# esw0116/DynaVSR

Hardware: AMD Instinct MI355X
Metric: inner-loop frames/sec/GPU (EDVR-M x4, 5x3x180x320): forward leg = BASELINE.json configs[1]; the inner MAML step and the per-frame pipeline are `inner_step` / `per_frame_pipeline` (higher is better)
Workload: dtype f32; 1 GPU; EDVR-M x4 forward (PCD deformable alignment + TSA fusion + reconstruction), clips of 1x5x3x180x320 -> 3x720x1280 (BASELINE.json configs[1]); one step = 2 clip(s) per GPU, one per HIP stream (adapt.super_resolve_video); clips_in_flight_per_gpu=2

## Files before the change

dynavsr_amd/_lib.py:

```python
import ctypes
import os
from ctypes import POINTER, Structure, c_char_p, c_float, c_int, c_longlong, c_size_t, c_void_p

import torch

_runtime = {"configured": False, "hw_queues": None, "effective": None}


def configure_runtime(hw_queues=6):
    if not _runtime["configured"]:
        user = os.environ.get("GPU_MAX_HW_QUEUES")
        late = torch.cuda.is_initialized()
        if user is None and not late:
            os.environ["GPU_MAX_HW_QUEUES"] = str(int(hw_queues))
        _runtime.update(configured=True, hw_queues=os.environ.get("GPU_MAX_HW_QUEUES"),
                        effective=(user is not None) or not late)
    return {"hw_queues": _runtime["hw_queues"], "effective": _runtime["effective"]}


def runtime_report(device=None):
    r = configure_runtime()
    overlaps = None
    if torch.cuda.is_available():
        with torch.cuda.device(device if device is not None else torch.cuda.current_device()):
# ... 101 lines not shown
        "dvsr_conv2d_backward": (I, [POINTER(Conv2dDesc), P, P, P, P, P, P, c_size_t, P]),
        "dvsr_mdcn_backward_workspace_bytes": (c_size_t, [I] * 10),
        "dvsr_mdcn_backward": (I, [P] * 10 + [I] * 12 + [P, c_size_t, P]),
        "dvsr_adam_step": (I, [POINTER(c_void_p)] * 4 + [POINTER(LL), I, F, F, F, F, F, I, P]),
        "dvsr_sgd_step": (I, [POINTER(c_void_p)] * 2 + [POINTER(LL), I, F, F, P]),
        "dvsr_replicate_tensors": (I, [POINTER(c_void_p)] * 2 + [POINTER(LL), I, I, P]),
        "dvsr_degrade_apply": (I, [P, P, P, I, I, I, I, I, I, I, I, I, P]),
        "dvsr_frame_metrics_workspace_bytes": (c_size_t, [I, I, I]),
        "dvsr_frame_metrics": (I, [P, P, I, I, I, F, F, P, P, P, c_size_t, P]),
        "dvsr_charbonnier_workspace_bytes": (c_size_t, []),
        "dvsr_charbonnier_forward": (I, [P, P, P, LL, F, P, c_size_t, P]),
        "dvsr_conv2d_packed_workspace_bytes": (c_size_t, [POINTER(Conv2dDesc)]),
        "dvsr_conv2d_forward_packed": (I, [POINTER(Conv2dDesc), P, c_size_t, P]),
        "dvsr_conv2d_dgrad_packed": (I, [POINTER(Conv2dDesc), P, P, P, c_size_t, P]),
        "dvsr_conv2d_packed_geometry": (I, [POINTER(Conv2dDesc), POINTER(ctypes.c_int * 4)]),
        "dvsr_conv2d_wgrad_geometry": (I, [POINTER(Conv2dDesc), I, I, POINTER(ctypes.c_int * 8)]),
        "dvsr_conv2d_wgrad_workspace_bytes": (c_size_t, [POINTER(Conv2dDesc), I]),
        "dvsr_conv2d_wgrad_bf16": (I, [POINTER(Conv2dDesc), P, P, P, P, c_size_t, P]),
        "dvsr_conv2d_wgrad_split3": (I, [POINTER(Conv2dDesc), P, P, P, P, c_size_t, P]),
        "dvsr_flow_warp_forward": (I, [P, P, P, I, I, I, I, LL, P]),
        "dvsr_flow_warp_backward": (I, [P, P, P, P, P, I, I, I, I, LL, P]),
        "dvsr_avgpool2_forward": (I, [P, P, LL, I, I, P]),
        "dvsr_avgpool2_backward": (I, [P, P, LL, I, I, I, P]),
        "dvsr_resize_bilinear_ac_forward": (I, [P, P, LL, I, I, I, I, F, LL, P]),
        "dvsr_resize_bilinear_ac_backward": (I, [P, P, LL, I, I, I, I, F, LL, P]),
        "dvsr_upsample_bicubic_ac_forward": (I, [P, P, LL, I, I, I, P]),
        "dvsr_upsample_bicubic_ac_backward": (I, [P, P, LL, I, I, I, P]),
        "dvsr_channel_affine": (I, [P, P, P, P, I, I, LL, LL, LL, I, P]),
        "dvsr_batchnorm_workspace_bytes": (c_size_t, [I]),
        "dvsr_batchnorm_forward": (I, [P] * 8 + [I, I, LL, I, F, F, I, P, c_size_t, P]),
# ... 10 lines not shown
        "dvsr_l1_tail_backward": (I, [P, P, P, F, P, LL, P]),
        "dvsr_charbonnier_backward": (I, [P, P, P, P, LL, F, P]),
        "dvsr_charbonnier_forward_grouped": (I, [P, P, P, LL, I, F, P, c_size_t, P]),
        "dvsr_charbonnier_backward_grouped": (I, [P, P, P, P, LL, I, F, P]),
        "dvsr_l1_tail_forward_grouped": (I, [P, P, P, F, P, LL, I, P, c_size_t, P]),
        "dvsr_l1_tail_backward_grouped": (I, [P, P, P, F, P, LL, I, P]),
        "dvsr_edvr_op_info": (I, [P, I, c_char_p, I, c_char_p, I, POINTER(ctypes.c_double),
                                  POINTER(ctypes.c_double)]),
        "dvsr_edvr_forward_timed": (I, [P, POINTER(c_void_p), P, P, P, c_size_t, P, POINTER(c_float)]),
        "dvsr_debug_mfma_peak": (LL, [P, I, I, I, I, P]),
        "dvsr_debug_mfma_shadow": (I, [P, P, I, I, I, I, I, P]),
        "dvsr_edvr_tensor_info": (I, [P, c_char_p, POINTER(LL), POINTER(LL)]),
        "dvsr_edvr_plan_work": (I, [P, POINTER(ctypes.c_double * 9)]),
        "dvsr_edvr_plan_work_nograd": (I, [P, POINTER(ctypes.c_double * 9)]),
        "dvsr_edvr_op_launch_count": (I, [P, I, I]),
        "dvsr_side_stream_overlaps": (I, [P]),
        "dvsr_edvr_op_output": (I, [P, I, I, POINTER(c_int), POINTER(LL), POINTER(LL)]),
        "dvsr_estimator_plan_work": (I, [P, POINTER(ctypes.c_double * 9)]),
        "dvsr_edvr_stream_create": (I, [POINTER(EdvrConfig), I, I, I, POINTER(c_void_p)]),
        "dvsr_edvr_stream_destroy": (None, [P]),
        "dvsr_edvr_stream_num_params": (I, [P]),
        "dvsr_edvr_stream_num_launches": (I, [P, I]),
        "dvsr_edvr_stream_cache_bytes": (c_size_t, [P]),
        "dvsr_edvr_stream_workspace_bytes": (c_size_t, [P]),
        "dvsr_edvr_stream_extract": (I, [P, POINTER(c_void_p), P, I, P, c_size_t, P, c_size_t, I, P]),
        "dvsr_edvr_stream_fuse": (I, [P, POINTER(c_void_p), POINTER(c_int), P, c_size_t, P, P, c_size_t, I, P]),
        "dvsr_frame_ingest": (I, [P, POINTER(FrameDesc), P, I, I, I, P]),
        "dvsr_frame_emit": (I, [P, I, I, P, POINTER(FrameDesc), F, F, P]),
        "dvsr_edvr_stream_extract_frame": (I, [P, POINTER(c_void_p), P, POINTER(FrameDesc), I, I, P, c_size_t, P, c_size_t, I,
                                               P]),
# ... 52 lines not shown
```

dynavsr_amd/csrc/conv2d_v2.hip:

```cpp
#include <algorithm>
#include <cmath>
#include <cstdlib>
#include <type_traits>

#include "common.h"
#include "kernels.h"
#include "small_grid.h"

namespace dvsr {

#ifdef DVSR_CONV_TRACE
#define DVSR_ABLATE(a) ((a).ablate)
#define DVSR_STAMP(i)                                                                              \
  do {                                                                                             \
    if (a.trace && threadIdx.x == 0) a.trace[(size_t)blockIdx.x * 64 + (i)] = __builtin_readcyclecounter(); \
  } while (0)
#else
#define DVSR_ABLATE(a) 0
#define DVSR_STAMP(i) \
  do {                \
  } while (0)
#endif

template <int KS, int S, int CC, int TH, int MT, int BF = 0>
struct Conv2Shape {
  static constexpr int TW = 32, KK = KS * KS, NT = TH / 4;
  static constexpr int IH = (TH - 1) * S + KS, IW = (TW - 1) * S + KS;
  static constexpr int PLANE = IH * IW, E = (PLANE + 255) / 256;
  static constexpr int KQ4 = BF ? CC / 16 : CC / 8;
  static constexpr int PIECES = BF == 2 ? 3 : 1;
  static constexpr int IN1 = KQ4 * PLANE * 8;
  static constexpr int IN_FLOATS = PIECES * IN1;
  static constexpr int HALF = KK * KQ4 * 2 * 32 * 4;
  static constexpr int W1 = MT * HALF;
  static constexpr bool AG = BF == 2;
  static constexpr int W_FLOATS = AG ? 0 : PIECES * W1;
  static constexpr int NPIECE = W_FLOATS / 256;
  static constexpr int BUF_FLOATS = IN_FLOATS + W_FLOATS;
  static constexpr size_t LDS_BYTES = (size_t)2 * BUF_FLOATS * sizeof(float);
};

__global__ void pack_weights_kernel(PackTable t) {
  const PackEntry& e = t.e[blockIdx.y];
  if (e.bf || has_own_pack_kernel(e.layout)) return;
  const int kq4 = e.CC / 8;
  const size_t per_chunk = (size_t)e.pch;
  const size_t total = (size_t)e.ncb * e.nchunks * per_chunk;
  for (size_t i = blockIdx.x * (size_t)blockDim.x + threadIdx.x; i < total;
       i += (size_t)gridDim.x * blockDim.x) {
    int r = (int)(i % per_chunk);
    const size_t ck = i / per_chunk;
    const int k = (int)(ck % e.nchunks), cb = (int)(ck / e.nchunks);
    const int j = r & 3; r >>= 2;
    const int lo = r & 31; r >>= 5;
// ... 100 lines not shown
  const int wave = __builtin_amdgcn_readfirstlane(tid >> 6);
  const int lo = lane & 31, hi = lane >> 5;
  const int Ctot = a.c0 + a.c1;
  const size_t HW = (size_t)a.H * a.W;
  const float* x0n = a.x0 + (size_t)n * a.x0_bs;
  const float* x1n = a.c1 ? a.x1 + (size_t)(n / a.x1_bdiv) * a.x1_bs : x0n;
  const size_t cstride0 = a.in_dil ? (size_t)a.Hs * a.Ws : HW;

  unsigned eoffb[E];
  int elds[E];
  bool evalid[E];
#pragma unroll
  for (int e = 0; e < E; ++e) {
    const int idx = tid + 256 * e;
    const int iy = idx / IW, ix = idx - iy * IW;
    elds[e] = (iy * 2) * IW + ix;
    const int gy = iy0 + iy, gx = ix0 + ix;
    bool ok = idx < PLANE && (unsigned)gy < (unsigned)a.H && (unsigned)gx < (unsigned)a.W;
    int off = gy * a.W + gx;
    if (a.in_ps) off = (2 * gy) * (2 * a.W) + 2 * gx;
    if (a.in_dil) {
      ok = ok && !((gy | gx) & 1) && (gy >> 1) < a.Hs && (gx >> 1) < a.Ws;
      off = (gy >> 1) * a.Ws + (gx >> 1);
    }
    eoffb[e] = ok ? (unsigned)off * 4u : 0u;
    evalid[e] = ok;
  }

  f32x16 acc[MT][NT];
#pragma unroll
  for (int i = 0; i < MT; ++i)
// ... 51 lines not shown
#pragma unroll
          for (int h2 = 0; h2 < 2; ++h2) {
            const bool ev = evalid[e];
            f32x4 v;
            if (BF == 2) {
              const int cb0 = k * CC + 16 * q + 8 * h2;
              bf16x8 p0, p1, p2;
#pragma unroll
              for (int i = 0; i < 8; ++i) {
                const float x = (ev && cb0 + i < Ctot) ? rin[16 * q + 8 * h2 + i][e] : 0.f;
                const __bf16 h = (__bf16)x;
                const float r1 = x - (float)h;
                const __bf16 m = (__bf16)r1;
                p0[i] = h; p1[i] = m; p2[i] = (__bf16)(r1 - (float)m);
              }
              float* dst = s_in + ((size_t)(q * IH * 2 * IW) + elds[e] + h2 * IW) * 4;
              *reinterpret_cast<f32x4*>(dst + Sh::IN1) = __builtin_bit_cast(f32x4, p1);
              *reinterpret_cast<f32x4*>(dst + 2 * Sh::IN1) = __builtin_bit_cast(f32x4, p2);
              v = __builtin_bit_cast(f32x4, p0);
            } else if (BF) {
              const int cb0 = k * CC + 16 * q + 8 * h2;
              bf16x8 hv;
#pragma unroll
              for (int i = 0; i < 8; ++i) hv[i] = (__bf16)((ev && cb0 + i < Ctot) ? rin[16 * q + 8 * h2 + i][e] : 0.f);
              v = __builtin_bit_cast(f32x4, hv);
            } else {
              const int cb0 = k * CC + 8 * q + h2;
              v = f32x4{(ev && cb0 < Ctot) ? rin[8 * q + h2][e] : 0.f,
                        (ev && cb0 + 2 < Ctot) ? rin[8 * q + 2 + h2][e] : 0.f,
                        (ev && cb0 + 4 < Ctot) ? rin[8 * q + 4 + h2][e] : 0.f,
                        (ev && cb0 + 6 < Ctot) ? rin[8 * q + 6 + h2][e] : 0.f};
            }
            *reinterpret_cast<f32x4*>(s_in + ((size_t)(q * IH * 2 * IW) + elds[e] + h2 * IW) * 4) = v;
          }
      }
    }
  };

  constexpr int NSTEP = KK * KQ4;
  constexpr int SPLIT = (3 * NSTEP) / 4;
  constexpr int RING = NSTEP % 3 == 0 ? 3 : 2;
  static_assert(!Sh::AG || (NSTEP % RING == 0 && KQ4 == 1), "the register ring of the global-A path needs NSTEP % RING == 0");
  constexpr int AD = 1;
  f32x4 Ag[Sh::AG ? RING : 1][MT][PIECES];
  auto load_a = [&](int k, int tap, int slot) {
    const float* b = wp_cb + (size_t)k * (PIECES * 2 * Sh::HALF) + tap * 256 + lane * 4;
#pragma unroll
    for (int op = 0; op < PIECES; ++op)
#pragma unroll
      for (int mt = 0; mt < MT; ++mt)
        Ag[slot][mt][op] = *reinterpret_cast<const f32x4*>(b + (op * 2 + mt) * Sh::HALF);
  };
  auto block = [&](int k, auto has_next_tag) {
    constexpr bool HAS_NEXT = decltype(has_next_tag)::value;
    const int buf = k & 1;
    const float* s_in = s_in0 + buf * Sh::BUF_FLOATS;
    const float* s_w = s_w0 + buf * Sh::BUF_FLOATS;
    if (k < 8) DVSR_STAMP(2 + 4 * k);
    if (HAS_NEXT && !Sh::AG) {
      issue_dma(k + 1, buf ^ 1);
      issue_halo(k + 1);
      __builtin_amdgcn_sched_barrier(0);
    }
    if (k < 8) DVSR_STAMP(3 + 4 * k);
    f32x4 A[2][Sh::AG ? 1 : MT][PIECES], Bv[Sh::AG ? 1 : 2][NT][PIECES];
    auto load_ops = [&](int step, int rb) {
      const int tap = step / KQ4, q = step - tap * KQ4;
      const int ty = tap / KS, tx = tap - ty * KS;
#pragma unroll
      for (int op = 0; op < PIECES; ++op) {
        if constexpr (!Sh::AG) {
#pragma unroll
          for (int mt = 0; mt < MT; ++mt)
            A[rb][mt][op] = *reinterpret_cast<const f32x4*>(
                s_w + op * Sh::W1 + ((size_t)((((mt * KK + tap) * KQ4 + q) * 2 + hi) * 32 + lo)) * 4);
        }
#pragma unroll
        for (int nt = 0; nt < NT; ++nt)
          Bv[rb][nt][op] = *reinterpret_cast<const f32x4*>(
              s_in + op * Sh::IN1 + ((size_t)(((q * IH + (NT * wave + nt) * S + ty) * 2 + hi) * IW + lo * S + tx)) * 4);
      }
    };
    auto load_b = [&](int step, int op) {
      const int ty = step / KS, tx = step - ty * KS;
#pragma unroll
      for (int nt = 0; nt < NT; ++nt)
        Bv[0][nt][op] = *reinterpret_cast<const f32x4*>(
            s_in + op * Sh::IN1 + ((size_t)((((NT * wave + nt) * S + ty) * 2 + hi) * IW + lo * S + tx)) * 4);
    };
    if constexpr (Sh::AG) { load_b(0, 2); load_b(0, 1); load_b(0, 0); }
    else load_ops(0, 0);
#pragma unroll
    for (int step = 0; step < NSTEP; ++step) {
      const int rb = step & 1;
      if constexpr (Sh::AG) {
        if (step + AD < NSTEP) load_a(k, step + AD, (step + AD) % RING);
        else if (HAS_NEXT) load_a(k + 1, step + AD - NSTEP, (step + AD) % RING);
        if (HAS_NEXT && step == 0) issue_halo(k + 1);
        __builtin_amdgcn_sched_barrier(0);
      }
      if (!Sh::AG && step + 1 < NSTEP) load_ops(step + 1, rb ^ 1);
      if (HAS_NEXT && step == SPLIT) {
        if (k < 8) DVSR_STAMP(4 + 4 * k);
        __builtin_amdgcn_sched_barrier(0);
        write_halo(k + 1, buf ^ 1);
        __builtin_amdgcn_sched_barrier(0);
        if (k < 8) DVSR_STAMP(5 + 4 * k);
      }
      if constexpr (BF == 2) {
        auto mm = [&](int pa, int pb) {
#pragma unroll
          for (int mt = 0; mt < MT; ++mt)
#pragma unroll
            for (int nt = 0; nt < NT; ++nt)
              acc[mt][nt] = __builtin_amdgcn_mfma_f32_32x32x16_bf16(
                  __builtin_bit_cast(bf16x8, Ag[step % RING][mt][pa]), __builtin_bit_cast(bf16x8, Bv[0][nt][pb]),
                  acc[mt][nt], 0, 0, 0);
        };
        mm(0, 2);
        if (step + 1 < NSTEP) { load_b(step + 1, 2); __builtin_amdgcn_sched_barrier(0); }
// ... 10 lines not shown
#pragma unroll
          for (int nt = 0; nt < NT; ++nt)
            acc[mt][nt] = __builtin_amdgcn_mfma_f32_32x32x16_bf16(__builtin_bit_cast(bf16x8, A[rb][mt][0]),
                                                                  __builtin_bit_cast(bf16x8, Bv[rb][nt][0]), acc[mt][nt],
                                                                  0, 0, 0);
      } else {
#pragma unroll
        for (int j = 0; j < 4; ++j)
#pragma unroll
          for (int mt = 0; mt < MT; ++mt)
#pragma unroll
            for (int nt = 0; nt < NT; ++nt)
              acc[mt][nt] = __builtin_amdgcn_mfma_f32_32x32x2f32(A[rb][mt][0][j], Bv[rb][nt][0][j], acc[mt][nt], 0, 0, 0);
      }
    }
    if (HAS_NEXT) __syncthreads();
  };

  DVSR_STAMP(0);
#ifdef DVSR_CONV_TRACE
  if (a.trace && threadIdx.x == 0) a.trace[(size_t)blockIdx.x * 64 + 60] = __builtin_amdgcn_s_memrealtime();
#endif
  issue_dma(0, 0);
  if constexpr (Sh::AG) {
#pragma unroll
    for (int i = 0; i < AD; ++i) load_a(0, i, i);
  }
  issue_halo(0);
  write_halo(0, 0);
  DVSR_STAMP(1);
// ... 3 lines not shown

  DVSR_STAMP(40);
  const TileOut t{a.y, wset_ptr(a.bias, a.b_gs, n, a.wdiv), a.res, a.act, a.ps, a.accum, a.Cout, a.Ho, a.Wo, a.gmask, a.gmask_act};
  store_mfma_tile<MT, NT>(acc, t, n, cbi * MT * 32, oy0, TH, ox0, oy0 + NT * wave, lo, hi);
#ifdef DVSR_CONV_TRACE
  DVSR_STAMP(41);
  __builtin_amdgcn_s_waitcnt(0);
  DVSR_STAMP(42);
  if (a.trace && threadIdx.x == 0) a.trace[(size_t)blockIdx.x * 64 + 61] = __builtin_amdgcn_s_memrealtime();
  if (a.trace && threadIdx.x == 0)
    a.trace[(size_t)blockIdx.x * 64 + 63] = __builtin_amdgcn_s_getreg((4) | (0 << 6) | (31 << 11));
#endif
}

template <int KS, int S, int CC, int TH, int MT, int BF = 0>
__global__ __launch_bounds__(256, (BF == 2 && TH == 4) ? 3 : 2) void conv2d_pipe_kernel(ConvK2 a) {
  extern __shared__ __attribute__((aligned(16))) float smem[];
  conv2d_pipe_item<KS, S, CC, TH, MT, BF>(a, blockIdx.x, smem);
}

template <int KS, int S, int CC, int TH, int MT, int BF = 0>
static int launch_conv2(ConvK2 k, hipStream_t st) {
  using Sh = Conv2Shape<KS, S, CC, TH, MT, BF>;
  auto kern = conv2d_pipe_kernel<KS, S, CC, TH, MT, BF>;
  static PerDeviceOnce attr_once;
  size_t lds = Sh::LDS_BYTES;
#ifdef DVSR_CONV_TRACE
  if (const char* e = getenv("DVSR_CONV_LDS")) lds = std::max(lds, (size_t)atol(e));
#endif
  set_dyn_lds_once(attr_once, (const void*)kern, lds);
  k.tiles_x = ceil_div(k.Wo, 32); k.tiles_y = ceil_div(k.Ho, TH); k.ntiles = k.tiles_x * k.tiles_y * k.N;
// ... 402 lines not shown
constexpr double W5_CHUNK_CYC = 4300.0, W5_FIXED_CYC = 17500.0;
WinoPick wino_f4_cost(const ConvShape& s, double cus) {
  const double f8 = wino_rounds_cost(s, cus, 8, 64, W5_CHUNK_CYC, W5_FIXED_CYC), f16 = wino_rounds_cost(s, cus, 16, 32, W5_CHUNK_CYC, W5_FIXED_CYC);
  return {f16 < f8 ? 16 : 8, std::min(f8, f16)};
}
constexpr double SHARED_LATENCY_BOUND = 1.05;
bool f4_occupies_less(const ConvShape& s, double cus, const WinoPick& f2, const WinoPick& f4) {
  const int ow2 = f2.th == 16 ? 16 : (f2.th == 8 ? 32 : 64), ow4 = f4.th == 16 ? 32 : 64;
  const double g2 = wino_workgroups(s, f2.th, ow2), g4 = wino_workgroups(s, f4.th, ow4);
  if (g2 > cus || g4 > cus) return false;
  ConvShape one = s;
  one.N = 1;
  if (2.0 * wino_workgroups(one, f2.th, ow2) <= cus || 2.0 * wino_workgroups(one, f4.th, ow4) > cus) return false;
  return g4 * f4.cost < g2 * f2.cost && f4.cost <= SHARED_LATENCY_BOUND * f2.cost;
}
}

double conv2_f4_occupied_cycles(int N, int Ho, int Wo, int Cout, int Ctot, int th) {
  const ConvShape s{3, 1, N, Ho, Wo, Cout, Ctot};
  return wino_workgroups(s, th, th == 16 ? 32 : 64) * ((Ctot / 8) * W5_CHUNK_CYC + W5_FIXED_CYC);
}

ConvGeo conv2_choose(int ks, int stride, int N, int Ho, int Wo, int Cout, int Ctot, ConvAllow allow) {
  const ConvShape s{ks, stride, N, Ho, Wo, Cout, Ctot};
  if (ks == 7 || ks == 9) return choose_row_split(s, allow);
  ConvGeo g;
  if (choose_ksplit(s, allow, &g)) return g;
  g = choose_direct_tile(s);
  if ((allow & ALLOW_DMA_HALO) && ks == 3 && stride == 1 && Wo % 4 == 0 && Ctot % 8 == 0) g.kernel = ConvKernel::DMA_HALO;
  const int wino_on = int_or(getenv("DVSR_CONV_WINO"), 1);
// ... 112 lines not shown
  }
  return DVSR_OK;
}

template <int KS, int S, int CC, int TH, int BF>
static int launch_conv2_mt(int mt, const ConvK2& k, hipStream_t st) {
  return mt == 2 ? launch_conv2<KS, S, CC, TH, 2, BF>(k, st) : launch_conv2<KS, S, CC, TH, 1, BF>(k, st);
}

int conv2d_packed_run(const dvsr_conv2d_desc& d, const float* wp, const ConvExtra& ex, const ConvGeo& geo,
                      hipStream_t st) {
  ConvK2 k;
  int rc = conv2d_packed_prepare(d, wp, ex, geo, &k);
  if (rc) return rc;
  if (geo.bf) {
    DVSR_REQUIRE((d.ks == 3 || (d.ks == 2 && geo.bf == 2)) && d.stride == 1 && geo.cc == 16 && (geo.th == 4 || (geo.bf == 2 && geo.th == 8)),
                 DVSR_ERR_UNSUPPORTED,
                 "conv2d_packed: the bf16 kernel exists for 3x3 (split: also 2x2) stride-1 convs with 16-channel chunks");
    const bool th8 = geo.th == 8;
    if (geo.bf == 2 && d.ks == 2)
      return th8 ? launch_conv2_mt<2, 1, 16, 8, 2>(geo.mt, k, st) : launch_conv2_mt<2, 1, 16, 4, 2>(geo.mt, k, st);
    if (geo.bf == 2) return th8 ? launch_conv2_mt<3, 1, 16, 8, 2>(geo.mt, k, st) : launch_conv2_mt<3, 1, 16, 4, 2>(geo.mt, k, st);
    return launch_conv2_mt<3, 1, 16, 4, 1>(geo.mt, k, st);
  }
  switch (geo.kernel) {
    case ConvKernel::WINO_F2: return conv2d_wino_launch(k, geo.th, st);
    case ConvKernel::WINO_F2_BF16: return conv2d_wino3_launch(k, geo.th, st);
    case ConvKernel::WINO_F4: return conv2d_wino5_launch(k, geo.th, st);
    case ConvKernel::ROW_SPLIT:
      if (d.ks == 7) return geo.mt == 2 ? launch_dmarow<7, 4, 2>(k, st) : launch_dmarow<7, 4, 1>(k, st);
      return geo.mt == 2 ? launch_dmarow<9, 4, 2>(k, st) : launch_dmarow<9, 4, 1>(k, st);
    case ConvKernel::DMA_HALO:
      if (geo.th != 4) break;
      return geo.mt == 2 ? launch_dma<4, 2>(k, st) : launch_dma<4, 1>(k, st);
// ... 78 lines not shown
  DVSR_REQUIRE(d && geo && (d->ks == 1 || d->ks == 3 || d->ks == 7 || d->ks == 9) && d->stride == 1 && d->pad == d->ks / 2,
               DVSR_ERR_INVALID, "conv2d_packed_geometry: 1x1 / 3x3 / 7x7 / 9x9 stride-1 descriptors only");
  const OpPack o = op_pack_for(*d, d->Cout, d->c0 + d->c1);
  geo[0] = o.geo.cc; geo[1] = o.geo.th; geo[2] = o.geo.mt; geo[3] = static_cast<int>(o.geo.kernel);
  return DVSR_OK;
}

extern "C" int dvsr_conv2d_forward_packed(const dvsr_conv2d_desc* d, void* workspace, size_t workspace_bytes,
                                          dvsr_stream_t stream) {
  DVSR_REQUIRE(d && d->x0 && d->w && d->y, DVSR_ERR_INVALID, "conv2d_forward_packed: null argument");
  DVSR_REQUIRE(d->pixel_shuffle == 0 || (d->pixel_shuffle == 2 && d->Cout % 4 == 0 && !d->res), DVSR_ERR_INVALID,
               "conv2d_forward_packed: pixel_shuffle needs Cout %% 4 == 0 and no residual");
  return op_run(*d, dvsr::ConvExtra(), d->Cout, d->c0 + d->c1, workspace, workspace_bytes, (hipStream_t)stream);
}

extern "C" int dvsr_conv2d_dgrad_packed(const dvsr_conv2d_desc* d, const float* gy, float* gx0, void* workspace,
                                        size_t workspace_bytes, dvsr_stream_t stream) {
  using namespace dvsr;
  DVSR_REQUIRE(d && gy && gx0 && d->w, DVSR_ERR_INVALID, "conv2d_dgrad_packed: null argument");
  DVSR_REQUIRE(d->c1 == 0 && d->pixel_shuffle == 0, DVSR_ERR_UNSUPPORTED, "conv2d_dgrad_packed: single plain input only");
  dvsr_conv2d_desc g = {};
  g.x0 = gy; g.w = d->w; g.y = gx0; g.N = d->N; g.c0 = d->Cout; g.Cout = d->c0; g.H = d->H; g.W = d->W; g.ks = d->ks;
  g.stride = 1; g.pad = d->ks / 2; g.act = ACT_NONE; g.x1_bdiv = 1;
  ConvExtra ex;
  ex.wt = 1; ex.w_ctot = d->c0; ex.w_coff = 0;
  return op_run(g, ex, d->c0, d->Cout, workspace, workspace_bytes, (hipStream_t)stream);
}
```

dynavsr_amd/csrc/engine.hip:

```cpp
#include <algorithm>
#include <cstdlib>
#include <string>
#include <vector>

#include "common.h"
#include "kernels.h"
#include "small_grid.h"

namespace dvsr {

enum { SP_ARENA = 0, SP_INPUT = 1, SP_OUTPUT = 2, SP_NONE = 3 };
struct T {
  int space = SP_NONE;
  size_t off = 0, numel = 0;
  bool valid() const { return space != SP_NONE; }
};

enum OpType { OP_CONV, OP_DCN, OP_UP, OP_POOL, OP_GATE, OP_BLEND, OP_ADD, OP_PAD, OP_MEANSUB, OP_ADDMEAN };

struct Op {
  OpType type;
  const char* name = "";
  T x0, x1, res, y, y2;
  int pw = -1, pb = -1;
// ... 139 lines not shown
    return g;
  };
  const bool plain = o.pad < 0 && !o.wmap && !p.cfg.bf16_mfma;
  const ConvAllow ks_ok = (plain && (c1 == 0 || c0 % 32 == 0) ? ALLOW_KSPLIT : ALLOW_NONE) |
                          (plain && c0 % 8 == 0 && c1 % 8 == 0 ? ALLOW_DMA_HALO | ALLOW_WINO : ALLOW_NONE);
  const ConvAllow fwd_ok = (o.ps == 0 || (o.ps == 2 && !o.res.valid())) ? ks_ok : without(ks_ok, ALLOW_WINO);
  auto whole = [&](const ConvGeo& g) {
    const size_t floats = conv2_pack_floats(ks, Cout, c0 + c1, g);
    return Op::Launch{{g, arena_alloc(p, "", floats * p.wsets).off, floats}, 0, c0 + c1, Op::WHOLE};
  };
  o.launches[FWD_GRAD] = {1, {whole(as_bf(conv2_choose(ks, o.stride, N, Ho, Wo, Cout, c0 + c1, fwd_ok), Ho, Wo, Cout))}};
  Op::LaunchList& nograd = o.launches[FWD_NOGRAD] = o.launches[FWD_GRAD];
  if ((fwd_ok & ALLOW_WINO) && !nograd.l[0].pack.geo.bf) {
    const ConvGeo g5 = conv2_choose(ks, o.stride, N, Ho, Wo, Cout, c0 + c1, fwd_ok | ALLOW_WINO_F4 | ALLOW_SHARED_DEVICE);
    if (g5.kernel == ConvKernel::WINO_F4) nograd.l[0] = whole(g5);
  }
  const Op::LaunchList pair = plan_hoist(o, p, fwd_ok, nograd.l[0]);
  if (pair.n) {
    o.pre = arena_alloc(p, "", (size_t)(N / o.x1_bdiv) * Cout * Ho * Wo);
    nograd = pair;
  }
  for (int which = 0; which < 2; ++which) {
    const int ci = which ? c1 : c0;
    if (!ci) continue;
    Op::PackSlot& dg = o.dgrad[which];
    dg.geo = as_bf(conv2_choose(ks, 1, N, o.H, o.W, ci, Cout, (!o.ps && o.stride == 1) ? ks_ok : ALLOW_NONE), o.H, o.W, ci, true);
    dg.floats = conv2_pack_floats(ks, ci, Cout, dg.geo);
    dg.off = p.dpack_floats;
    p.dpack_floats += dg.floats * p.wsets;
  }
// ... 965 lines not shown
      *kind = "mdcn";
      break;
    }
    case OP_UP: *bytes = 4.0 * o.planes * o.H * o.W * (1.0 + o.S * o.S); *kind = "upsample"; break;
    case OP_POOL: *bytes = 4.0 * o.planes * o.H * o.W * 1.5; *kind = "pool"; break;
    case OP_GATE: *bytes = 4.0 * ((double)o.gB * o.gN * o.gC * o.gHW * 3 + (double)o.gB * o.gC * o.gHW +
                                 (double)o.gB * o.gN * o.gHW); *kind = "tsa_gate"; break;
    case OP_BLEND: *bytes = 4.0 * o.y.numel * 4; *kind = "tsa_blend"; break;
    case OP_ADD: *bytes = 4.0 * o.y.numel * 3; *kind = "add"; break;
    case OP_PAD: *bytes = 4.0 * ((double)o.N * o.c0 * o.H * o.W + (double)o.y.numel); *kind = "pad"; break;
    case OP_MEANSUB: *bytes = 4.0 * o.y.numel * 3; *kind = "meansub"; break;
    case OP_ADDMEAN: *bytes = 4.0 * o.y.numel * 2; *kind = "addmean"; break;
  }
}

extern "C" int dvsr_edvr_op_info(const dvsr_edvr_plan* p, int index, char* kind, int kind_cap,
                                 char* name, int name_cap, double* flops, double* bytes) {
  DVSR_REQUIRE(p && kind && name && flops && bytes && index >= 0 && index < (int)p->ops.size(),
               DVSR_ERR_INVALID, "edvr_op_info: bad argument");
  const char* k;
  op_work(p->ops[index], &k, flops, bytes);
  snprintf(kind, kind_cap, "%s", k);
  if (p->ops[index].type == OP_CONV)
  {
    const ConvGeo& g = p->ops[index].launches[FWD_NOGRAD].primary().pack.geo;
    snprintf(name, name_cap, "%s[%d/%d/%d%s]", p->ops[index].name, g.cc, g.th, g.mt, kernel_tag(g.kernel));
  }
  else
    snprintf(name, name_cap, "%s", p->ops[index].name);
  return DVSR_OK;
}

extern "C" int dvsr_edvr_op_launch_count(const dvsr_edvr_plan* p, int index, int nograd) {
  if (!p || index < 0 || index >= (int)p->ops.size()) return -1;
  const Op& o = p->ops[index];
  return o.type == OP_CONV ? o.launches[nograd ? FWD_NOGRAD : FWD_GRAD].n : 1;
}

static int plan_work(const dvsr_edvr_plan* p, double* out9, FwdMode mode) {
  DVSR_REQUIRE(p && out9, DVSR_ERR_INVALID, "edvr_plan_work: null argument");
  double fa = 0, fe = 0, ba = 0, be = 0, fby = 0, f32p[2] = {0, 0}, bfp[2] = {0, 0};
// ... 436 lines not shown
```

dynavsr_amd/csrc/kernels.h:

```cpp
#pragma once
#include "../../include/dynavsr_hip.h"
#include "common.h"

namespace dvsr {

struct ConvExtra {
  int wt = 0;
  int w_ctot = 0, w_coff = 0;
  int in_ps = 0;
  int in_dil = 0, Hs = 0, Ws = 0;
  int accum = 0;
  const float* gmask = nullptr;
  int gmask_act = 0;
  int wdiv = 1; long long w_gs = 0; int b_gs = 0;
};
int conv2d_run(const dvsr_conv2d_desc& d, const ConvExtra& ex, hipStream_t st);

int mdcn_forward_run(const float* x, const float* off, long long off_bs, const float* msk,
                     long long msk_bs, int mask_logit, const float* w, const float* b, float* out,
                     int N, int C, int H, int W, int Cout, int kh, int kw, int stride, int pad,
                     int dil, int groups, int dg, int act, hipStream_t st);

enum class ConvKernel : int {
  REG = 0,
// ... 8 lines not shown
  DMA_ORDER = 1,
  ROW_SPLIT = 2,
  WINO_F2 = 3,
  WINO_F2_BF16 = 4,
  WINO_F4 = 5,
  DCN_SPLIT = 6,
};
constexpr PackLayout pack_layout(ConvKernel k) { return static_cast<PackLayout>(static_cast<int>(k)); }
constexpr bool is_winograd(ConvKernel k) { return k == ConvKernel::WINO_F2 || k == ConvKernel::WINO_F2_BF16 || k == ConvKernel::WINO_F4; }
constexpr bool on_bf16_split(ConvKernel k) { return k == ConvKernel::WINO_F2_BF16 || k == ConvKernel::WINO_F4; }
constexpr bool needs_dma_halo_inputs(ConvKernel k) { return k == ConvKernel::DMA_HALO || is_winograd(k); }
constexpr double multiplies_per_output_ratio(ConvKernel k) { return k == ConvKernel::WINO_F4 ? 0.25 : (is_winograd(k) ? 16.0 / 36.0 : 1.0); }
constexpr const char* kernel_tag(ConvKernel k) {
  return k == ConvKernel::WINO_F4 ? "w5" : (k == ConvKernel::WINO_F2_BF16 ? "w3" : (k == ConvKernel::WINO_F2 ? "w" : (k == ConvKernel::REG ? "" : "d")));
}
constexpr bool has_own_pack_kernel(PackLayout l) { return static_cast<int>(l) >= static_cast<int>(PackLayout::WINO_F2); }

struct PackEntry {
  const float* w; float* P;
  int Cout, Ctot, KK, CC, wt, w_ctot, w_coff, ncb, nchunks, pch;
  int bf = 0;
  PackLayout layout = PackLayout::INTERLEAVED;
};
struct PackTable {
  int n;
  PackEntry e[48];
};
int pack_weights_run(const PackTable& t, hipStream_t st);
struct ConvGeo { int cc, th, mt; int bf = 0; ConvKernel kernel = ConvKernel::REG; };
enum ConvAllow : int {
// ... 6 lines not shown
  ALLOW_ONLY_F4 = 32,
};
constexpr ConvAllow operator|(ConvAllow a, ConvAllow b) { return static_cast<ConvAllow>(static_cast<int>(a) | static_cast<int>(b)); }
constexpr ConvAllow without(ConvAllow a, ConvAllow b) { return static_cast<ConvAllow>(static_cast<int>(a) & ~static_cast<int>(b)); }
ConvGeo conv2_choose(int ks, int stride, int N, int Ho, int Wo, int Cout, int Ctot, ConvAllow allow = ALLOW_KSPLIT);
size_t conv2_pack_floats(int ks, int Cout, int Ctot, int cc, int bf, PackLayout layout);
PackEntry conv2_pack_entry(const float* w, float* P, int ks, int Cout, int Ctot, int cc, int bf, PackLayout layout, int wt = 0,
                           int w_ctot = 0, int w_coff = 0);
inline size_t conv2_pack_floats(int ks, int Cout, int Ctot, const ConvGeo& g) {
  return conv2_pack_floats(ks, Cout, Ctot, g.cc, g.bf, pack_layout(g.kernel));
}
inline PackEntry conv2_pack_entry(const float* w, float* P, int ks, int Cout, int Ctot, const ConvGeo& g, int wt = 0, int w_ctot = 0,
                                  int w_coff = 0) {
  return conv2_pack_entry(w, P, ks, Cout, Ctot, g.cc, g.bf, pack_layout(g.kernel), wt, w_ctot, w_coff);
}
double conv2_f4_occupied_cycles(int N, int Ho, int Wo, int Cout, int Ctot, int th);
int pack_weights_wino_run(const PackTable& t, hipStream_t st);
int pack_weights_wino3_run(const PackTable& t, hipStream_t st);
int pack_weights_wino5_run(const PackTable& t, hipStream_t st);
int conv2d_packed_run(const dvsr_conv2d_desc& d, const float* wp, const ConvExtra& ex, const ConvGeo& geo,
                      hipStream_t st);

bool conv1x1_dual_ok(const float* x, const float* w0, const float* w1, const float* y0, const float* y1, int Cin, long long HW);
int conv1x1_dual_run(const float* x, const float* w0, const float* b0, const float* w1, const float* b1, float* y0, float* y1,
                     int N, int Cin, int HW, int act, hipStream_t st, int wdiv = 1, long long w_gs = 0, int b_gs = 0);
int conv3x3_small_cout_run(const float* x, const float* w, const float* bias, const float* res, float* y, int N,
                           int C, int H, int W, int Cout, int act, hipStream_t st, int wdiv = 1, long long w_gs = 0,
                           int b_gs = 0);

struct WgradReduceEntry {
// ... 156 lines not shown
```

dynavsr_amd/engine.py:

```python
import ctypes
import threading

import torch

from . import _lib as L

_plans = {}
_GEOMETRY_ENV = ("DVSR_CONV_WINO", "DVSR_CONV_WINO3", "DVSR_CONV_WINO5", "DVSR_CONV_V1", "DVSR_EST_SPLIT", "DVSR_EST_SPLIT2", "DVSR_FUSE_ACT_BWD",
                 "DVSR_BWD_STREAMS", "DVSR_PCD_HOIST")
_PROCESS_ENV = ("DVSR_CONV_LDS", "DVSR_CONV_LAST_MFMA", "DVSR_SPLIT_TH8_FROM", "DVSR_WGRAD_SPLIT3",
                "DVSR_WGRAD_WIDE", "DVSR_WGRAD_S3V", "DVSR_WGRAD_S3_KYS_BELOW", "DVSR_WGRAD_S3_WGS", "DVSR_WGRAD_S3W", "DVSR_DCN_FWD", "DVSR_DCN_BWD",
                "DVSR_EST_FUSE_PAD", "DVSR_FUSE_RES_BWD", "DVSR_BWD_FORK_EVERY", "DVSR_BWD_PROBE", "DVSR_TSA_DUAL", "DVSR_TSA_V",
                "DVSR_DEGRADE_GENERIC", "DVSR_UP2")
_process_env_seen = None


def _check_process_env():
    import os
    import warnings
    global _process_env_seen
    now = tuple(os.environ.get(k) for k in _PROCESS_ENV)
    if _process_env_seen is None:
        _process_env_seen = now
        return
    for k, a, b in zip(_PROCESS_ENV, _process_env_seen, now):
        if a != b:
            warnings.warn("dynavsr_amd: %s=%r now, but the native library read %r when the first plan of this process was built "
                          "and keeps that value (switches of this kind are read once per process: set them before the first "
# ... 58 lines not shown
        ia, off, n = ctypes.c_int(), ctypes.c_longlong(), ctypes.c_longlong()
        L.check(L.lib().dvsr_edvr_op_output(self._h, index, which, ctypes.byref(ia), ctypes.byref(off), ctypes.byref(n)),
                "dvsr_edvr_op_output")
        if not ia.value:
            return None
        return ws.view(torch.float32)[off.value:off.value + n.value]

    def op_info(self):
        out = []
        kind, name = ctypes.create_string_buffer(32), ctypes.create_string_buffer(64)
        fl, by = ctypes.c_double(), ctypes.c_double()
        for i in range(self.n_launches):
            L.check(L.lib().dvsr_edvr_op_info(self._h, i, kind, 32, name, 64, ctypes.byref(fl),
                                              ctypes.byref(by)), "dvsr_edvr_op_info")
            out.append((kind.value.decode(), name.value.decode(), fl.value, by.value))
        return out

    def tensor(self, ws, name, shape=None):
        off, n = ctypes.c_longlong(), ctypes.c_longlong()
        L.check(L.lib().dvsr_edvr_tensor_info(self._h, name.encode(), ctypes.byref(off),
                                              ctypes.byref(n)), "dvsr_edvr_tensor_info")
        t = ws.view(torch.float32)[off.value:off.value + n.value]
        return t.view(shape) if shape is not None else t

    def __del__(self):
        try:
            if self._h:
                L.lib().dvsr_edvr_plan_destroy(self._h)
        except Exception:
            pass
# ... 416 lines not shown
```

include/dynavsr_hip.h:

```cpp
#ifndef DYNAVSR_HIP_H_
#define DYNAVSR_HIP_H_

#include <stddef.h>

#ifdef __cplusplus
extern "C" {
#endif

#define DVSR_OK 0
#define DVSR_ERR_INVALID (-1)
#define DVSR_ERR_UNSUPPORTED (-2)
#define DVSR_ERR_WORKSPACE (-3)
#define DVSR_ERR_HIP (-4)

#define DVSR_ACT_NONE 0
#define DVSR_ACT_LRELU 1
#define DVSR_ACT_RELU 2

typedef void* dvsr_stream_t;

const char* dvsr_last_error(void);
int dvsr_version(void);

int dvsr_mdcn_forward(const float* x, const float* offset, const float* mask, const float* w,
// ... 78 lines not shown
int dvsr_edvr_num_launches(const dvsr_edvr_plan* plan);
size_t dvsr_edvr_workspace_bytes(const dvsr_edvr_plan* plan, int need_grad);
int dvsr_edvr_forward(const dvsr_edvr_plan* plan, const float* const* params, const float* x,
                      float* out, void* workspace, size_t workspace_bytes, dvsr_stream_t stream);
int dvsr_edvr_forward_packed(const dvsr_edvr_plan* plan, const float* const* params, const float* x,
                             float* out, void* workspace, size_t workspace_bytes, dvsr_stream_t stream);
int dvsr_edvr_backward(const dvsr_edvr_plan* plan, const float* const* params, const float* x,
                       const float* grad_out, float* const* grad_params, float* grad_x, void* workspace,
                       size_t workspace_bytes, dvsr_stream_t stream);
int dvsr_edvr_num_backward_launches(const dvsr_edvr_plan* plan);
int dvsr_edvr_op_info(const dvsr_edvr_plan* plan, int index, char* kind, int kind_cap, char* name,
                      int name_cap, double* flops, double* bytes);
int dvsr_edvr_plan_work(const dvsr_edvr_plan* plan, double* out9);
int dvsr_edvr_plan_work_nograd(const dvsr_edvr_plan* plan, double* out9);
int dvsr_edvr_op_launch_count(const dvsr_edvr_plan* plan, int index, int nograd);
int dvsr_side_stream_overlaps(dvsr_stream_t stream);
int dvsr_edvr_op_output(const dvsr_edvr_plan* plan, int index, int which, int* in_arena, long long* offset_floats,
                        long long* numel);
int dvsr_edvr_forward_timed(const dvsr_edvr_plan* plan, const float* const* params, const float* x,
                            float* out, void* workspace, size_t workspace_bytes,
                            dvsr_stream_t stream, float* op_ms);
long long dvsr_debug_mfma_peak(float* out, int blocks, int iters, int nacc, int lds_bytes, dvsr_stream_t stream);
int dvsr_debug_mfma_shadow(long long* cycles, float* out, int blocks, int iters, int nv, int kind, int acc,
                           dvsr_stream_t stream);
int dvsr_edvr_tensor_info(const dvsr_edvr_plan* plan, const char* name, long long* offset_floats,
                          long long* numel);

#define DVSR_STREAM_MAX_FRAMES 16
typedef struct dvsr_edvr_stream dvsr_edvr_stream;
int dvsr_edvr_stream_create(const dvsr_edvr_config* cfg, int H, int W, int slots, dvsr_edvr_stream** out);
// ... 116 lines not shown
                                      int groups, float eps, dvsr_stream_t stream);

int dvsr_l1_tail_forward(const float* x, const float* y, const float* base, float weight, float* loss, long long n,
                         void* workspace, size_t workspace_bytes, dvsr_stream_t stream);
int dvsr_l1_tail_backward(const float* x, const float* y, const float* grad_loss, float weight, float* gx, long long n,
                          dvsr_stream_t stream);
int dvsr_l1_tail_forward_grouped(const float* x, const float* y, const float* base, float weight, float* loss, long long n,
                                 int groups, void* workspace, size_t workspace_bytes, dvsr_stream_t stream);
int dvsr_l1_tail_backward_grouped(const float* x, const float* y, const float* grad_loss, float weight, float* gx,
                                  long long n, int groups, dvsr_stream_t stream);

size_t dvsr_conv2d_packed_workspace_bytes(const dvsr_conv2d_desc* d);
int dvsr_conv2d_forward_packed(const dvsr_conv2d_desc* d, void* workspace, size_t workspace_bytes, dvsr_stream_t stream);
int dvsr_conv2d_dgrad_packed(const dvsr_conv2d_desc* d, const float* gy, float* gx0, void* workspace,
                             size_t workspace_bytes, dvsr_stream_t stream);
int dvsr_conv2d_packed_geometry(const dvsr_conv2d_desc* d, int geo[4]);

int dvsr_conv2d_wgrad_bf16(const dvsr_conv2d_desc* d, const float* gy, float* gw, float* gb, void* workspace,
                           size_t workspace_bytes, dvsr_stream_t stream);
int dvsr_conv2d_wgrad_split3(const dvsr_conv2d_desc* d, const float* gy, float* gw, float* gb, void* workspace,
                             size_t workspace_bytes, dvsr_stream_t stream);

int dvsr_conv2d_wgrad_geometry(const dvsr_conv2d_desc* d, int mode, int groups, int geo[8]);
size_t dvsr_conv2d_wgrad_workspace_bytes(const dvsr_conv2d_desc* d, int groups);

int dvsr_flow_warp_forward(const float* x, const float* flow, float* out, int N, int C, int H, int W,
                           long long out_bstride, dvsr_stream_t stream);
int dvsr_flow_warp_backward(const float* x, const float* flow, const float* grad_out, float* grad_x, float* grad_flow,
                            int N, int C, int H, int W, long long gout_bstride, dvsr_stream_t stream);
int dvsr_avgpool2_forward(const float* x, float* y, long long planes, int H, int W, dvsr_stream_t stream);
// ... 64 lines not shown
```

Before: 260.9 frames/s.

## Route stride-2 3x3 no-grad convs through split-bf16 MFMA kernel with deinterleaved LDS

Extends the split-bf16 (three-piece) MFMA conv kernel to 3x3 stride-2 convolutions. Input columns are stored in LDS deinterleaved by parity so strided taps read contiguous columns, and the kernel drops to single-buffered LDS to fit the larger footprint. The engine picks this path for no-grad stride-2 convs only at the two measured pyramid sizes, when a cost model favours it over the fp32 kernel. The trade is lost double-buffer overlap and hard-coded shape gating; debug tags and a standalone test entry point are also added.

```diff
diff --git a/dynavsr_amd/_lib.py b/dynavsr_amd/_lib.py
--- a/dynavsr_amd/_lib.py
+++ b/dynavsr_amd/_lib.py
@@ -139,6 +139,8 @@
         "dvsr_conv2d_forward_packed": (I, [POINTER(Conv2dDesc), P, c_size_t, P]),
         "dvsr_conv2d_dgrad_packed": (I, [POINTER(Conv2dDesc), P, P, P, c_size_t, P]),
         "dvsr_conv2d_packed_geometry": (I, [POINTER(Conv2dDesc), POINTER(ctypes.c_int * 4)]),
+        "dvsr_conv2d_stride2_workspace_bytes": (c_size_t, [POINTER(Conv2dDesc), I]),
+        "dvsr_conv2d_forward_stride2": (I, [POINTER(Conv2dDesc), I, P, c_size_t, P]),
         "dvsr_conv2d_wgrad_geometry": (I, [POINTER(Conv2dDesc), I, I, POINTER(ctypes.c_int * 8)]),
         "dvsr_conv2d_wgrad_workspace_bytes": (c_size_t, [POINTER(Conv2dDesc), I]),
         "dvsr_conv2d_wgrad_bf16": (I, [POINTER(Conv2dDesc), P, P, P, P, c_size_t, P]),
@@ -179,6 +181,7 @@
         "dvsr_edvr_plan_work": (I, [P, POINTER(ctypes.c_double * 9)]),
         "dvsr_edvr_plan_work_nograd": (I, [P, POINTER(ctypes.c_double * 9)]),
         "dvsr_edvr_op_launch_count": (I, [P, I, I]),
+        "dvsr_edvr_op_tag": (I, [P, I, I, c_char_p, I]),
         "dvsr_side_stream_overlaps": (I, [P]),
         "dvsr_edvr_op_output": (I, [P, I, I, POINTER(c_int), POINTER(LL), POINTER(LL)]),
         "dvsr_estimator_plan_work": (I, [P, POINTER(ctypes.c_double * 9)]),
diff --git a/dynavsr_amd/csrc/conv2d_v2.hip b/dynavsr_amd/csrc/conv2d_v2.hip
--- a/dynavsr_amd/csrc/conv2d_v2.hip
+++ b/dynavsr_amd/csrc/conv2d_v2.hip
@@ -29,7 +29,9 @@
   static constexpr int PLANE = IH * IW, E = (PLANE + 255) / 256;
   static constexpr int KQ4 = BF ? CC / 16 : CC / 8;
   static constexpr int PIECES = BF == 2 ? 3 : 1;
-  static constexpr int IN1 = KQ4 * PLANE * 8;
+  static constexpr bool DEINT = BF == 2 && S == 2;
+  static constexpr int COFF = 36, RW = DEINT ? COFF + TW : IW;
+  static constexpr int IN1 = KQ4 * IH * 2 * RW * 4;
   static constexpr int IN_FLOATS = PIECES * IN1;
   static constexpr int HALF = KK * KQ4 * 2 * 32 * 4;
   static constexpr int W1 = MT * HALF;
@@ -37,7 +39,8 @@
   static constexpr int W_FLOATS = AG ? 0 : PIECES * W1;
   static constexpr int NPIECE = W_FLOATS / 256;
   static constexpr int BUF_FLOATS = IN_FLOATS + W_FLOATS;
-  static constexpr size_t LDS_BYTES = (size_t)2 * BUF_FLOATS * sizeof(float);
+  static constexpr int NBUF = DEINT ? 1 : 2;
+  static constexpr size_t LDS_BYTES = (size_t)NBUF * BUF_FLOATS * sizeof(float);
 };
 
 __global__ void pack_weights_kernel(PackTable t) {
@@ -168,7 +171,7 @@
   for (int e = 0; e < E; ++e) {
     const int idx = tid + 256 * e;
     const int iy = idx / IW, ix = idx - iy * IW;
-    elds[e] = (iy * 2) * IW + ix;
+    elds[e] = (iy * 2) * Sh::RW + (Sh::DEINT ? (ix & 1) * Sh::COFF + (ix >> 1) : ix);
     const int gy = iy0 + iy, gx = ix0 + ix;
     bool ok = idx < PLANE && (unsigned)gy < (unsigned)a.H && (unsigned)gx < (unsigned)a.W;
     int off = gy * a.W + gx;
@@ -250,7 +253,7 @@
                 const __bf16 m = (__bf16)r1;
                 p0[i] = h; p1[i] = m; p2[i] = (__bf16)(r1 - (float)m);
               }
-              float* dst = s_in + ((size_t)(q * IH * 2 * IW) + elds[e] + h2 * IW) * 4;
+              float* dst = s_in + ((size_t)(q * IH * 2 * Sh::RW) + elds[e] + h2 * Sh::RW) * 4;
               *reinterpret_cast<f32x4*>(dst + Sh::IN1) = __builtin_bit_cast(f32x4, p1);
               *reinterpret_cast<f32x4*>(dst + 2 * Sh::IN1) = __builtin_bit_cast(f32x4, p2);
               v = __builtin_bit_cast(f32x4, p0);
@@ -267,7 +270,7 @@
                         (ev && cb0 + 4 < Ctot) ? rin[8 * q + 4 + h2][e] : 0.f,
                         (ev && cb0 + 6 < Ctot) ? rin[8 * q + 6 + h2][e] : 0.f};
             }
-            *reinterpret_cast<f32x4*>(s_in + ((size_t)(q * IH * 2 * IW) + elds[e] + h2 * IW) * 4) = v;
+            *reinterpret_cast<f32x4*>(s_in + ((size_t)(q * IH * 2 * Sh::RW) + elds[e] + h2 * Sh::RW) * 4) = v;
           }
       }
     }
@@ -289,17 +292,18 @@
   };
   auto block = [&](int k, auto has_next_tag) {
     constexpr bool HAS_NEXT = decltype(has_next_tag)::value;
-    const int buf = k & 1;
+    const int buf = Sh::NBUF == 2 ? (k & 1) : 0, nbuf = Sh::NBUF == 2 ? (buf ^ 1) : 0;
     const float* s_in = s_in0 + buf * Sh::BUF_FLOATS;
     const float* s_w = s_w0 + buf * Sh::BUF_FLOATS;
     if (k < 8) DVSR_STAMP(2 + 4 * k);
     if (HAS_NEXT && !Sh::AG) {
-      issue_dma(k + 1, buf ^ 1);
+      issue_dma(k + 1, nbuf);
       issue_halo(k + 1);
       __builtin_amdgcn_sched_barrier(0);
     }
     if (k < 8) DVSR_STAMP(3 + 4 * k);
     f32x4 A[2][Sh::AG ? 1 : MT][PIECES], Bv[Sh::AG ? 1 : 2][NT][PIECES];
+    auto bcol = [&](int tx) { return Sh::DEINT ? (tx & 1) * Sh::COFF + (tx >> 1) + lo : lo * S + tx; };
     auto load_ops = [&](int step, int rb) {
       const int tap = step / KQ4, q = step - tap * KQ4;
       const int ty = tap / KS, tx = tap - ty * KS;
@@ -314,7 +318,7 @@
 #pragma unroll
         for (int nt = 0; nt < NT; ++nt)
           Bv[rb][nt][op] = *reinterpret_cast<const f32x4*>(
-              s_in + op * Sh::IN1 + ((size_t)(((q * IH + (NT * wave + nt) * S + ty) * 2 + hi) * IW + lo * S + tx)) * 4);
+              s_in + op * Sh::IN1 + ((size_t)(((q * IH + (NT * wave + nt) * S + ty) * 2 + hi) * Sh::RW + bcol(tx))) * 4);
       }
     };
     auto load_b = [&](int step, int op) {
@@ -322,7 +326,7 @@
 #pragma unroll
       for (int nt = 0; nt < NT; ++nt)
         Bv[0][nt][op] = *reinterpret_cast<const f32x4*>(
-            s_in + op * Sh::IN1 + ((size_t)((((NT * wave + nt) * S + ty) * 2 + hi) * IW + lo * S + tx)) * 4);
+            s_in + op * Sh::IN1 + ((size_t)((((NT * wave + nt) * S + ty) * 2 + hi) * Sh::RW + bcol(tx))) * 4);
     };
     if constexpr (Sh::AG) { load_b(0, 2); load_b(0, 1); load_b(0, 0); }
     else load_ops(0, 0);
@@ -336,10 +340,10 @@
         __builtin_amdgcn_sched_barrier(0);
       }
       if (!Sh::AG && step + 1 < NSTEP) load_ops(step + 1, rb ^ 1);
-      if (HAS_NEXT && step == SPLIT) {
+      if (HAS_NEXT && step == SPLIT && Sh::NBUF == 2) {
         if (k < 8) DVSR_STAMP(4 + 4 * k);
         __builtin_amdgcn_sched_barrier(0);
-        write_halo(k + 1, buf ^ 1);
+        write_halo(k + 1, nbuf);
         __builtin_amdgcn_sched_barrier(0);
         if (k < 8) DVSR_STAMP(5 + 4 * k);
       }
@@ -380,6 +384,10 @@
               acc[mt][nt] = __builtin_amdgcn_mfma_f32_32x32x2f32(A[rb][mt][0][j], Bv[rb][nt][0][j], acc[mt][nt], 0, 0, 0);
       }
     }
+    if (HAS_NEXT && Sh::NBUF == 1) {
+      __syncthreads();
+      write_halo(k + 1, 0);
+    }
     if (HAS_NEXT) __syncthreads();
   };
 
@@ -413,7 +421,7 @@
 }
 
 template <int KS, int S, int CC, int TH, int MT, int BF = 0>
-__global__ __launch_bounds__(256, (BF == 2 && TH == 4) ? 3 : 2) void conv2d_pipe_kernel(ConvK2 a) {
+__global__ __launch_bounds__(256, (BF == 2 && TH == 4 && S == 1) ? 3 : 2) void conv2d_pipe_kernel(ConvK2 a) {
   extern __shared__ __attribute__((aligned(16))) float smem[];
   conv2d_pipe_item<KS, S, CC, TH, MT, BF>(a, blockIdx.x, smem);
 }
@@ -846,6 +854,23 @@
   if (2.0 * wino_workgroups(one, f2.th, ow2) <= cus || 2.0 * wino_workgroups(one, f4.th, ow4) > cus) return false;
   return g4 * f4.cost < g2 * f2.cost && f4.cost <= SHARED_LATENCY_BOUND * f2.cost;
 }
+}
+
+bool conv2_s2_split_choose(int Ho, int Wo, int Cout, int Ctot, ConvGeo* g) {
+  static const bool on = [] { const char* v = getenv("DVSR_CONV_S2_SPLIT"); return !(v && v[0] == '0'); }();
+  if (!on || Ctot % 16 != 0 || Cout % 32 != 0) return false;
+  static const int timed[][2] = {{90, 160}, {45, 80}};
+  bool measured = false;
+  for (const auto& t : timed) measured = measured || (Ho == t[0] && Wo == t[1]);
+  if (!measured) return false;
+  const ConvShape one{3, 2, 1, Ho, Wo, Cout, Ctot};
+  const ConvGeo f = choose_direct_tile(one);
+  const double fp32 = conv2_pipe_cost(f.th, f.mt, f.cc, one) * (Ctot / 8.0);
+  const int mt = mt1_wins(16, one) ? 1 : 2;
+  const double split = conv2_pipe_cost(4, mt, 16, one) * (6.0 * 32.0 / (8.0 * 64.0)) * (Ctot / 16.0);
+  if (split >= fp32) return false;
+  *g = ConvGeo{16, 4, mt, 2, ConvKernel::REG};
+  return true;
 }
 
 double conv2_f4_occupied_cycles(int N, int Ho, int Wo, int Cout, int Ctot, int th) {
@@ -988,10 +1013,13 @@
   int rc = conv2d_packed_prepare(d, wp, ex, geo, &k);
   if (rc) return rc;
   if (geo.bf) {
-    DVSR_REQUIRE((d.ks == 3 || (d.ks == 2 && geo.bf == 2)) && d.stride == 1 && geo.cc == 16 && (geo.th == 4 || (geo.bf == 2 && geo.th == 8)),
+    const bool s2 = d.stride == 2 && d.ks == 3 && geo.bf == 2 && geo.th == 4 && !ex.in_ps && !ex.in_dil;
+    DVSR_REQUIRE((d.ks == 3 || (d.ks == 2 && geo.bf == 2)) && (d.stride == 1 || s2) && geo.cc == 16 && (geo.th == 4 || (geo.bf == 2 && geo.th == 8)),
                  DVSR_ERR_UNSUPPORTED,
-                 "conv2d_packed: the bf16 kernel exists for 3x3 (split: also 2x2) stride-1 convs with 16-channel chunks");
+                 "conv2d_packed: the bf16 kernel exists for 3x3 (split: also 2x2, and 3x3 stride 2 on 4-row tiles) stride-1 convs with "
+                 "16-channel chunks (ks=%d stride=%d th=%d)", d.ks, d.stride, geo.th);
     const bool th8 = geo.th == 8;
+    if (s2) return launch_conv2_mt<3, 2, 16, 4, 2>(geo.mt, k, st);
     if (geo.bf == 2 && d.ks == 2)
       return th8 ? launch_conv2_mt<2, 1, 16, 8, 2>(geo.mt, k, st) : launch_conv2_mt<2, 1, 16, 4, 2>(geo.mt, k, st);
     if (geo.bf == 2) return th8 ? launch_conv2_mt<3, 1, 16, 8, 2>(geo.mt, k, st) : launch_conv2_mt<3, 1, 16, 4, 2>(geo.mt, k, st);
@@ -1100,6 +1128,34 @@
   return op_run(*d, dvsr::ConvExtra(), d->Cout, d->c0 + d->c1, workspace, workspace_bytes, (hipStream_t)stream);
 }
 
+static dvsr::ConvGeo s2_geo(const dvsr_conv2d_desc& d, int split_mt) {
+  using namespace dvsr;
+  if (split_mt) return ConvGeo{16, 4, split_mt, 2, ConvKernel::REG};
+  return conv2_choose(3, 2, d.N, (d.H - 1) / 2 + 1, (d.W - 1) / 2 + 1, d.Cout, d.c0, ALLOW_NONE);
+}
+extern "C" size_t dvsr_conv2d_stride2_workspace_bytes(const dvsr_conv2d_desc* d, int split_mt) {
+  if (!d || split_mt < 0 || split_mt > 2) return 0;
+  return dvsr::conv2_pack_floats(3, d->Cout, d->c0, s2_geo(*d, split_mt)) * sizeof(float);
+}
+extern "C" int dvsr_conv2d_forward_stride2(const dvsr_conv2d_desc* d, int split_mt, void* workspace, size_t workspace_bytes,
+                                           dvsr_stream_t stream) {
+  using namespace dvsr;
+  DVSR_REQUIRE(d && d->x0 && d->w && d->y && workspace, DVSR_ERR_INVALID, "conv2d_forward_stride2: null argument");
+  DVSR_REQUIRE(d->ks == 3 && d->stride == 2 && d->pad == 1 && d->c1 == 0 && !d->pixel_shuffle && !d->pre && split_mt >= 0 && split_mt <= 2,
+               DVSR_ERR_UNSUPPORTED, "conv2d_forward_stride2: a 3x3 / stride 2 / pad 1 convolution of one input, split_mt 0..2 (ks=%d stride=%d "
+               "pad=%d c1=%d split_mt=%d)", d->ks, d->stride, d->pad, d->c1, split_mt);
+  const ConvGeo geo = s2_geo(*d, split_mt);
+  const size_t floats = conv2_pack_floats(3, d->Cout, d->c0, geo);
+  DVSR_REQUIRE(workspace_bytes >= floats * sizeof(float), DVSR_ERR_WORKSPACE, "conv2d_forward_stride2: workspace %zu < %zu bytes",
+               workspace_bytes, floats * sizeof(float));
+  PackTable t;
+  t.n = 1;
+  t.e[0] = conv2_pack_entry(d->w, (float*)workspace, 3, d->Cout, d->c0, geo);
+  int rc = pack_weights_run(t, (hipStream_t)stream);
+  if (rc) return rc;
+  return conv2d_packed_run(*d, (const float*)workspace, ConvExtra(), geo, (hipStream_t)stream);
+}
+
 extern "C" int dvsr_conv2d_dgrad_packed(const dvsr_conv2d_desc* d, const float* gy, float* gx0, void* workspace,
                                         size_t workspace_bytes, dvsr_stream_t stream) {
   using namespace dvsr;
diff --git a/dynavsr_amd/csrc/engine.hip b/dynavsr_amd/csrc/engine.hip
--- a/dynavsr_amd/csrc/engine.hip
+++ b/dynavsr_amd/csrc/engine.hip
@@ -177,6 +177,10 @@
   if ((fwd_ok & ALLOW_WINO) && !nograd.l[0].pack.geo.bf) {
     const ConvGeo g5 = conv2_choose(ks, o.stride, N, Ho, Wo, Cout, c0 + c1, fwd_ok | ALLOW_WINO_F4 | ALLOW_SHARED_DEVICE);
     if (g5.kernel == ConvKernel::WINO_F4) nograd.l[0] = whole(g5);
+  }
+  if (ks == 3 && o.stride == 2 && o.pad < 0 && !o.wmap && !p.use_v1 && !nograd.l[0].pack.geo.bf && c1 == 0 && !o.ps) {
+    ConvGeo gs;
+    if (conv2_s2_split_choose(Ho, Wo, Cout, c0, &gs)) nograd.l[0] = whole(gs);
   }
   const Op::LaunchList pair = plan_hoist(o, p, fwd_ok, nograd.l[0]);
   if (pair.n) {
@@ -1172,6 +1176,18 @@
   }
 }
 
+static void conv_tag(const Op& o, FwdMode mode, char* tag, int cap) {
+  const ConvGeo& g = o.launches[mode].primary().pack.geo;
+  const bool s2_split = g.bf == 2 && o.stride == 2;
+  snprintf(tag, cap, "[%d/%d/%d%s]", g.cc, g.th, g.mt, s2_split ? S2_SPLIT_TAG : kernel_tag(g.kernel));
+}
+extern "C" int dvsr_edvr_op_tag(const dvsr_edvr_plan* p, int index, int nograd, char* tag, int tag_cap) {
+  DVSR_REQUIRE(p && tag && tag_cap > 0 && index >= 0 && index < (int)p->ops.size(), DVSR_ERR_INVALID, "edvr_op_tag: bad argument");
+  tag[0] = 0;
+  if (p->ops[index].type == OP_CONV) conv_tag(p->ops[index], nograd ? FWD_NOGRAD : FWD_GRAD, tag, tag_cap);
+  return DVSR_OK;
+}
+
 extern "C" int dvsr_edvr_op_info(const dvsr_edvr_plan* p, int index, char* kind, int kind_cap,
                                  char* name, int name_cap, double* flops, double* bytes) {
   DVSR_REQUIRE(p && kind && name && flops && bytes && index >= 0 && index < (int)p->ops.size(),
@@ -1181,8 +1197,9 @@
   snprintf(kind, kind_cap, "%s", k);
   if (p->ops[index].type == OP_CONV)
   {
-    const ConvGeo& g = p->ops[index].launches[FWD_NOGRAD].primary().pack.geo;
-    snprintf(name, name_cap, "%s[%d/%d/%d%s]", p->ops[index].name, g.cc, g.th, g.mt, kernel_tag(g.kernel));
+    char tag[24];
+    conv_tag(p->ops[index], FWD_NOGRAD, tag, sizeof tag);
+    snprintf(name, name_cap, "%s%s", p->ops[index].name, tag);
   }
   else
     snprintf(name, name_cap, "%s", p->ops[index].name);
diff --git a/dynavsr_amd/csrc/kernels.h b/dynavsr_amd/csrc/kernels.h
--- a/dynavsr_amd/csrc/kernels.h
+++ b/dynavsr_amd/csrc/kernels.h
@@ -46,6 +46,7 @@
 constexpr const char* kernel_tag(ConvKernel k) {
   return k == ConvKernel::WINO_F4 ? "w5" : (k == ConvKernel::WINO_F2_BF16 ? "w3" : (k == ConvKernel::WINO_F2 ? "w" : (k == ConvKernel::REG ? "" : "d")));
 }
+constexpr const char* S2_SPLIT_TAG = "s3";
 constexpr bool has_own_pack_kernel(PackLayout l) { return static_cast<int>(l) >= static_cast<int>(PackLayout::WINO_F2); }
 
 struct PackEntry {
@@ -82,6 +83,7 @@
                                   int w_coff = 0) {
   return conv2_pack_entry(w, P, ks, Cout, Ctot, g.cc, g.bf, pack_layout(g.kernel), wt, w_ctot, w_coff);
 }
+bool conv2_s2_split_choose(int Ho, int Wo, int Cout, int Ctot, ConvGeo* g);
 double conv2_f4_occupied_cycles(int N, int Ho, int Wo, int Cout, int Ctot, int th);
 int pack_weights_wino_run(const PackTable& t, hipStream_t st);
 int pack_weights_wino3_run(const PackTable& t, hipStream_t st);
diff --git a/dynavsr_amd/engine.py b/dynavsr_amd/engine.py
--- a/dynavsr_amd/engine.py
+++ b/dynavsr_amd/engine.py
@@ -11,7 +11,7 @@
 _PROCESS_ENV = ("DVSR_CONV_LDS", "DVSR_CONV_LAST_MFMA", "DVSR_SPLIT_TH8_FROM", "DVSR_WGRAD_SPLIT3",
                 "DVSR_WGRAD_WIDE", "DVSR_WGRAD_S3V", "DVSR_WGRAD_S3_KYS_BELOW", "DVSR_WGRAD_S3_WGS", "DVSR_WGRAD_S3W", "DVSR_DCN_FWD", "DVSR_DCN_BWD",
                 "DVSR_EST_FUSE_PAD", "DVSR_FUSE_RES_BWD", "DVSR_BWD_FORK_EVERY", "DVSR_BWD_PROBE", "DVSR_TSA_DUAL", "DVSR_TSA_V",
-                "DVSR_DEGRADE_GENERIC", "DVSR_UP2")
+                "DVSR_DEGRADE_GENERIC", "DVSR_UP2", "DVSR_CONV_S2_SPLIT")
 _process_env_seen = None
 
 
@@ -100,6 +100,13 @@
             L.check(L.lib().dvsr_edvr_op_info(self._h, i, kind, 32, name, 64, ctypes.byref(fl),
                                               ctypes.byref(by)), "dvsr_edvr_op_info")
             out.append((kind.value.decode(), name.value.decode(), fl.value, by.value))
+        return out
+
+    def op_tags(self, nograd=True):
+        buf, out = ctypes.create_string_buffer(32), []
+        for i in range(self.n_launches):
+            L.check(L.lib().dvsr_edvr_op_tag(self._h, i, int(nograd), buf, 32), "dvsr_edvr_op_tag")
+            out.append(buf.value.decode())
         return out
 
     def tensor(self, ws, name, shape=None):
diff --git a/include/dynavsr_hip.h b/include/dynavsr_hip.h
--- a/include/dynavsr_hip.h
+++ b/include/dynavsr_hip.h
@@ -116,6 +116,7 @@
 int dvsr_edvr_plan_work(const dvsr_edvr_plan* plan, double* out9);
 int dvsr_edvr_plan_work_nograd(const dvsr_edvr_plan* plan, double* out9);
 int dvsr_edvr_op_launch_count(const dvsr_edvr_plan* plan, int index, int nograd);
+int dvsr_edvr_op_tag(const dvsr_edvr_plan* plan, int index, int nograd, char* tag, int tag_cap);
 int dvsr_side_stream_overlaps(dvsr_stream_t stream);
 int dvsr_edvr_op_output(const dvsr_edvr_plan* plan, int index, int which, int* in_arena, long long* offset_floats,
                         long long* numel);
@@ -262,6 +263,8 @@
 int dvsr_conv2d_forward_packed(const dvsr_conv2d_desc* d, void* workspace, size_t workspace_bytes, dvsr_stream_t stream);
 int dvsr_conv2d_dgrad_packed(const dvsr_conv2d_desc* d, const float* gy, float* gx0, void* workspace,
                              size_t workspace_bytes, dvsr_stream_t stream);
+size_t dvsr_conv2d_stride2_workspace_bytes(const dvsr_conv2d_desc* d, int split_mt);
+int dvsr_conv2d_forward_stride2(const dvsr_conv2d_desc* d, int split_mt, void* workspace, size_t workspace_bytes, dvsr_stream_t stream);
 int dvsr_conv2d_packed_geometry(const dvsr_conv2d_desc* d, int geo[4]);
 
 int dvsr_conv2d_wgrad_bf16(const dvsr_conv2d_desc* d, const float* gy, float* gw, float* gb, void* workspace,
```

After: 262.3 frames/s (median of 6 runs). No clear change (+0.5%).
